# Jaureguy760/HaploHyped-VarAwareML

Measured on AMD Instinct MI355X. Metric: variants/sec encode+compress, 3M-variant x 2.5k-sample VCF, higher is better.
Workload: dtype u8

## Files before the change

### haplohyped_varawareml_amd/csrc/lz4bits.hip

```cpp
#include "common.h"

#define BP_N 4096
#ifndef BP_MAXONES
#define BP_MAXONES 636
#endif
#ifndef BP_STAGE
#define BP_STAGE 576
#endif
#ifndef BP_WAVES
#define BP_WAVES 7
#endif
#define BP_QCAP 100
#ifndef BP_MAXONES_EXC
#define BP_MAXONES_EXC 540
#endif
#ifndef BP_STAGE_EXC
#define BP_STAGE_EXC 448
#endif
template <bool EXC> struct BpCfg {
    static constexpr uint32_t MAXONES = EXC ? BP_MAXONES_EXC : BP_MAXONES;
    static constexpr uint32_t STAGE = EXC ? BP_STAGE_EXC : BP_STAGE;
    static constexpr uint32_t PTRASH = MAXONES + 7;
};
#define BP_HLOG 6
#define BP_GAPCLIP 40
#define BP_MINM 6
#define BP_TMIN 4
#define BP_BACK 64
#define BP_STEPS 16
#define BP_PICK 3
#define BP_LAZY_MIN 3
#ifdef BP_MARKS
#define BP_MARK(name) asm volatile("; ==MARK " name)
#else
#define BP_MARK(name)
#endif
#ifndef BP_SKIP
#define BP_SKIP 0
#endif
#define BP_MFLIMIT (BP_N - 12)
#define BP_MATCHLIMIT (BP_N - 5)

template <bool CHAIN, bool EXC> struct BpLds {
    uint32_t bm[132];
    uint32_t xm[EXC ? 132 : 1];
    uint32_t cls[EXC ? 24 : 1];
    uint32_t tab[1 << BP_HLOG];
    uint8_t flag[72];
    uint16_t wpre[64];
    uint16_t P[BpCfg<EXC>::MAXONES + 8];
    uint16_t chain[CHAIN ? BpCfg<EXC>::MAXONES + 8 : 4];
    uint32_t gbw[(BpCfg<EXC>::MAXONES + 16) / 4];
    uint2 queue[BP_QCAP + 1];
    uint8_t stage[BpCfg<EXC>::STAGE + 8];
};

__device__ __forceinline__ uint2 bp_entry(uint32_t E, uint32_t msr, bool onM, bool onT, uint32_t rs, uint32_t re, uint32_t off)
{
    return make_uint2(E | ((msr & 0x1FFFu) << 13) | (onM ? 1u << 26 : 0u) | (onT ? 1u << 27 : 0u) | ((rs - E) << 28), re | (off << 13));
}

__device__ __forceinline__ uint32_t bp_bits(const uint32_t *bm, uint32_t q)
{
    const uint32_t i = q >> 5;
    const uint32_t lo = bm[i], hi = bm[i + 1];
    return __builtin_amdgcn_alignbit(hi, lo, q & 31u);
}

__device__ __forceinline__ uint32_t bp_gap4(const uint32_t *gbw, uint32_t i)
{
    const uint32_t w = i >> 2;
    return __builtin_amdgcn_alignbit(gbw[w + 1u], gbw[w], (i & 3u) << 3);
}

__device__ __forceinline__ uint32_t bp_len_ext(uint32_t x) { return __umul24(x + 240u, 32897u) >> 23; }

template <bool EXC> __device__ __forceinline__ uint32_t bp_lit(uint32_t b, uint32_t x, uint32_t k)
{
    const uint32_t v = (b >> k) & 1u;
    return EXC ? (((x >> k) & 1u) ? 0xF7u : v) : v;
}

#define BP_FENCE() asm volatile("" ::: "memory")
#define BP_FORGET(x) asm volatile("" : "+v"(x))
#ifndef BP_EMITSKIP
#define BP_EMITSKIP 0
#endif
template <bool EXC, bool TR, typename OUT>
__device__ __forceinline__ void bp_put_entry(const uint32_t *bm, const uint32_t *xm, OUT out, uint32_t tr, uint32_t at, uint32_t pe, bool on1, uint32_t ll1,
                                             uint32_t ml1, uint32_t off1, bool on2, bool lit2, uint32_t ml2, uint32_t lane)
{
    if (BP_EMITSKIP == 3) return;
    const uint32_t llx1 = bp_len_ext(ll1), mlx1 = on1 ? bp_len_ext(ml1) : 0u, mlx2 = on2 ? bp_len_ext(ml2) : 0u, ll2 = lit2 ? 1u : 0u;
    auto put = [&](bool p, uint32_t a, uint32_t v) {
        if (TR) out[p ? a : tr] = (uint8_t)v;
        else if (p) out[a] = (uint8_t)v;
    };
    const uint32_t lit = at + 1u + llx1, o1 = lit + ll1;
    const uint32_t at2 = o1 + 2u + mlx1, o2 = at2 + 1u + ll2;
    if (__builtin_expect(__builtin_amdgcn_ballot_w64((llx1 > 1u) | (mlx1 > 1u) | (mlx2 > 1u)) != 0ull, 0)) {
        auto more = [&](uint32_t a, uint32_t v, uint32_t nx) {
            uint32_t r = v - 15u - 255u;
#pragma clang loop unroll(disable) vectorize(disable) interleave(disable)
            for (uint32_t k = 1; k < nx; ++k) {
                out[a + k] = (uint8_t)(k + 1u == nx ? r : 255u);
                r -= 255u;
            }
        };
        more(at + 1u, ll1, llx1);
        more(o1 + 2u, ml1, mlx1);
        more(o2 + 2u, ml2, mlx2);
    }
    put(on2, at2, (ll2 << 4) | (ml2 < 15u ? ml2 : 15u));
    put(lit2, at2 + 1u, 0u);
    put(on2, o2, 1u);
    put(on2, o2 + 1u, 0u);
    put(mlx2 != 0u, o2 + 2u, mlx2 == 1u ? ml2 - 15u : 255u);
    put(on1, at, ((ll1 < 15u ? ll1 : 15u) << 4) | (ml1 < 15u ? ml1 : 15u));
    put(llx1 != 0u, at + 1u, llx1 == 1u ? ll1 - 15u : 255u);
    put(on1, o1, off1 & 0xFFu);
    put(on1, o1 + 1u, off1 >> 8);
    put(mlx1 != 0u, o1 + 2u, mlx1 == 1u ? ml1 - 15u : 255u);
    if (BP_EMITSKIP != 1) {
        const uint32_t b = bp_bits(bm, pe), x = EXC ? bp_bits(xm, pe) : 0u;
        const uint32_t nsm = ll1 <= 6u ? ll1 : 0u;
#pragma unroll
        for (uint32_t k = 0; k < 6u; ++k) put(k < nsm, lit + k, bp_lit<EXC>(b, x, k));
        unsigned long long big = BP_EMITSKIP == 2 ? 0ull : __builtin_amdgcn_ballot_w64(ll1 > 6u);
        while (big != 0ull) {
            const int l = __builtin_ctzll(big);
            big &= big - 1ull;
            const uint32_t n = (uint32_t)__builtin_amdgcn_readlane((int)ll1, l);
            const uint32_t src = (uint32_t)__builtin_amdgcn_readlane((int)pe, l);
            const uint32_t dst = (uint32_t)__builtin_amdgcn_readlane((int)lit, l);
            for (uint32_t k = lane; k < n; k += 64u) out[dst + k] = (uint8_t)bp_lit<EXC>(bp_bits(bm, src + k), EXC ? bp_bits(xm, src + k) : 0u, 0u);
        }
    }
}

__device__ __forceinline__ void bp_flush(const uint8_t *stage, uint8_t *__restrict__ dst, uint32_t n, uint32_t lane)
{
    struct __attribute__((packed)) PU32 {
        uint32_t v;
    };
    const uint32_t nd = n >> 2;
    for (uint32_t i = lane; i < nd; i += 64u) reinterpret_cast<PU32 *>(dst + 4u * i)->v = reinterpret_cast<const uint32_t *>(stage)[i];
    const uint32_t t = (nd << 2) + lane;
    if (t < n) dst[t] = stage[t];
}

struct BpOut {
    uint32_t prev_end, gop, sop;
};

template <bool EXC, typename LDS>
__device__ __forceinline__ BpOut bp_emit_batch(LDS &S, const uint32_t *bm, uint8_t *__restrict__ out, uint32_t n, uint32_t qn, BpOut st, uint32_t lane)
{
    const uint32_t *xm = S.xm;
    uint32_t prev_end = st.prev_end, gop = st.gop, sop = st.sop;
    const bool have = lane < n;
    uint2 en = S.queue[lane];
    en.x = have ? en.x : 0u;
    en.y = have ? en.y : 0u;
    const uint32_t E = en.x & 0x1FFFu, msr = (en.x >> 13) & 0x1FFFu, rs = E + (en.x >> 28), re = en.y & 0x1FFFu, off = en.y >> 13;
    const bool onM = (en.x >> 26) & 1u;
    bool onT = (en.x >> 27) & 1u;
    {
        uint32_t nx = S.queue[lane + 1u].x;
        nx = lane + 1u < qn ? nx : 0u;
        const uint32_t nmsr = (nx >> 13) & 0x1FFFu;
        const bool nM = (nx >> 26) & 1u;
        uint32_t nbk = nM && nmsr <= re ? re - nmsr : 0u;
        const uint32_t zt = re - rs;
        nbk = nbk < zt ? nbk : zt;
        onT = onT && zt - nbk >= BP_TMIN;
    }
    const uint32_t F0 = onT ? re : E;
    uint32_t Fp = (uint32_t)__builtin_amdgcn_update_dpp(0, (int)F0, 0x138 , 0xf, 0xf, false);
    Fp = lane ? Fp : prev_end;
    const uint32_t F = (onM || onT) ? F0 : Fp;
    uint32_t pe = (uint32_t)__builtin_amdgcn_update_dpp(0, (int)F, 0x138 , 0xf, 0xf, false);
    pe = lane ? pe : prev_end;
    prev_end = (uint32_t)__builtin_amdgcn_readlane((int)F, (int)(n - 1u));
    const uint32_t ms = msr > pe ? msr : pe;
    const bool on1 = onM | onT, on2 = onM & onT;
    const uint32_t s1 = onM ? ms : rs, e1 = onM ? E : re;
    uint32_t ll1 = on1 ? s1 - pe : 0u, ml1 = e1 - s1 - 4u;
    const uint32_t off1 = onM ? off : 1u;
    const bool lit2 = on2 & (rs != E);
    uint32_t ml2 = re - rs - 4u;
    const uint32_t sz = (on1 ? 3u + bp_len_ext(ll1) + ll1 + bp_len_ext(ml1) : 0u) + (on2 ? 3u + (lit2 ? 1u : 0u) + bp_len_ext(ml2) : 0u);
    const uint32_t sincl = wave_scan_sum_dpp(sz, lane);
    const uint32_t total = (uint32_t)__builtin_amdgcn_readlane((int)sincl, 63);
    BP_MARK("sizes_done");
    if (__builtin_expect(sop + total > BpCfg<EXC>::STAGE, 0)) {
        bp_flush(S.stage, out + gop, sop, lane);
        gop += sop;
        sop = 0;
    }
    const uint32_t at = sincl - sz;
    BP_FORGET(ll1);
    BP_FORGET(ml1);
    BP_FORGET(ml2);
    if (__builtin_expect(total > BpCfg<EXC>::STAGE, 0)) {
        bp_put_entry<EXC, false>(bm, xm, out + gop, 0u, at, pe, on1, ll1, ml1, off1, on2, lit2, ml2, lane);
        gop += total;
    } else {
        bp_put_entry<EXC, true>(bm, xm, S.stage + sop, BpCfg<EXC>::STAGE - sop, at, pe, on1, ll1, ml1, off1, on2, lit2, ml2, lane);
        sop += total;
    }
    return BpOut{prev_end, gop, sop};
}


__device__ __forceinline__ void bp_probe_salu()
{
#ifdef BP_PROBE_SALU
#pragma unroll
    for (int pr = 0; pr < BP_PROBE_SALU; ++pr) asm volatile("s_mov_b32 s90, 0" ::: "s90");
#endif
}

__device__ __forceinline__ void bp_probe_valu()
{
#ifdef BP_PROBE_VALU
    uint32_t pv;
#pragma unroll
    for (int pr = 0; pr < BP_PROBE_VALU; ++pr) asm volatile("v_mov_b32 %0, 0" : "=v"(pv));
#endif
}

__device__ __forceinline__ uint32_t bp_probe_handoff(uint8_t *__restrict__ scratch, uint64_t sidx, uint64_t slot_bytes, uint32_t op, uint32_t lane)
{
#ifdef BP_PROBE_HANDOFF
    asm volatile("s_waitcnt vmcnt(0)" ::: "memory");
    uint32_t old = 0;
    if (lane == 0) old = atomicAdd(reinterpret_cast<uint32_t *>(scratch + (sidx & ~255ull) * slot_bytes + slot_bytes - 8u), 1u);
    old = (uint32_t)__builtin_amdgcn_readfirstlane((int)old);
    op += old == 0xFFFFFFF0u ? 1u : 0u;
#endif
    return op;
}

template <bool EXC, typename LDS>
__device__ __forceinline__ uint32_t bp_list_half(LDS &S, uint16_t *P, uint32_t w, uint32_t x, uint32_t at, uint32_t base)
{
    while (__builtin_amdgcn_ballot_w64(w != 0u) != 0ull) {
        const bool on = w != 0u;
        const uint32_t bpos = (uint32_t)__builtin_ctz(w | 0x80000000u);
        if (EXC && on && ((x >> bpos) & 1u)) atomicOr(&S.cls[at >> 5], 1u << (at & 31u));
        P[on ? at : BpCfg<EXC>::PTRASH] = (uint16_t)(base + bpos);
        at += on ? 1u : 0u;
        w &= w - 1u;
    }
    return at;
}

template <bool EXC, typename LDS>
__device__ __forceinline__ void bp_list_ones(LDS &S, uint16_t *P, uint16_t *wpre, uint32_t wlo, uint32_t whi, uint32_t xlo, uint32_t xhi, uint32_t incl,
                                             uint32_t cnt, uint32_t m, uint32_t lane)
{
    wpre[lane] = (uint16_t)(incl - cnt);
    BP_FENCE();
    P[lane == 0u ? 0u : BpCfg<EXC>::PTRASH] = 0;
    const uint32_t base = 64u * lane + 1u;
    const uint32_t at = bp_list_half<EXC>(S, P, wlo, xlo, incl - cnt + 1u, base);
    bp_list_half<EXC>(S, P, whi, xhi, at, base + 32u);
    P[lane < 4u ? m + 1u + lane : BpCfg<EXC>::PTRASH] = (uint16_t)(BP_N + 1);
    BP_FENCE();
}

template <bool EXC, typename LDS>
__device__ __forceinline__ void bp_gap_bytes(LDS &S, const uint16_t *P, uint32_t m, uint32_t lane)
{
    uint8_t *gb = reinterpret_cast<uint8_t *>(S.gbw);
    for (uint32_t i = lane; i < m + 8u; i += 64u) {
        const uint32_t i1 = i + 1u < BpCfg<EXC>::PTRASH ? i + 1u : BpCfg<EXC>::PTRASH;
        uint32_t g = (uint32_t)P[i1] - (uint32_t)P[i1 - 1u] - 1u;
        g = g < 255u ? g : 255u;
        gb[i] = (uint8_t)(i < m ? g : 255u);
    }
    BP_FENCE();
}

template <typename LDS>
__device__ __forceinline__ void bp_clear_table(LDS &S, uint32_t lane)
{
#pragma unroll
    for (int k = 0; k < (1 << BP_HLOG) / 64; ++k) S.tab[64 * k + lane] = 0u;
}

struct BpOne {
    int j, q;
    uint32_t jj, q1, qn1, qp1;
    uint32_t c5a;
    bool valid, can;
};

template <int DEPTH, bool EXC, typename LDS>
__device__ __forceinline__ BpOne bp_lane_one(LDS &S, const uint16_t *P, int jw, uint32_t m, uint32_t lane)
{
    BpOne o;
    o.j = jw + (int)lane;
    o.valid = o.j < (int)m;
    o.jj = o.valid ? (uint32_t)(o.j + 1) : 0u;
    o.q1 = P[o.jj], o.qn1 = P[o.jj + 1u];
    o.qp1 = o.jj ? P[o.jj - 1u] : 0u;
    o.q = (int)o.q1 - 1;
    o.can = DEPTH > 0 && o.valid && o.j >= 0 && o.q + 12 <= BP_N;
    o.c5a = EXC ? (bp_bits(S.cls, o.jj) & 31u) : 0u;
    return o;
}

template <bool CHAIN, bool EXC, typename LDS>
__device__ __forceinline__ uint32_t bp_table_insert(LDS &S, BpOne o)
{
    uint32_t jc1 = 0;
    if (o.can) {
        const uint32_t g1 = o.qn1 - o.q1;
        const uint32_t idx = (g1 < BP_GAPCLIP ? g1 : BP_GAPCLIP) ^ ((EXC && (o.c5a & 1u)) ? 63u : 0u);
        jc1 = atomicExch(&S.tab[idx], (uint32_t)(o.j + 1));
        if (CHAIN) S.chain[o.jj] = (uint16_t)jc1;
    }
    BP_FENCE();
    return jc1;
}

struct BpPick {
    int best;
    uint32_t bjq, bk;
    uint32_t a4;
};

template <int DEPTH, bool EXC, typename LDS>
__device__ __forceinline__ BpPick bp_pick(LDS &S, bool can, uint32_t jj, uint32_t c5a, uint32_t jc1)
{
    constexpr bool CHAIN = DEPTH > 1;
    const uint32_t a4 = bp_gap4(S.gbw, jj);
    const uint8_t *gbb = reinterpret_cast<const uint8_t *>(S.gbw);
    const uint32_t fa = jj ? (uint32_t)gbb[jj - 1u] : 0u;
    const uint32_t na4 = ~a4;
    const uint32_t stop4 = ((na4 - 0x01010101u) & ~na4 & 0x80808080u) | 0xFF000000u;
    int best = -1;
    uint32_t bjq = 0, bk = 0;
#pragma unroll 1
    for (int left = DEPTH; left > 0; --left) {
        const bool have = can && jc1 != 0u;
        if (__builtin_amdgcn_ballot_w64(have) == 0ull) break;
        const uint32_t jq = have ? jc1 : 1u;
        const uint32_t b4 = bp_gap4(S.gbw, jq);
        const uint32_t fb = (uint32_t)gbb[jq - 1u];
        uint32_t nextc = 0;
        if (CHAIN) nextc = S.chain[jq];
        const uint32_t x = (a4 ^ b4) | stop4;
        uint32_t k = (uint32_t)__builtin_ctz(x) >> 3;
        bool same = true;
        if (EXC) {
            const uint32_t xc = c5a ^ (bp_bits(S.cls, jq) & 31u);
            same = (xc & 1u) == 0u;
            const uint32_t tv = (uint32_t)__builtin_ctz((xc >> 1) | 8u);
            k = k < tv ? k : tv;
        }
        const uint32_t below = (1u << (8u * k)) - 1u;
        const uint32_t sumg = __builtin_amdgcn_sad_u8(a4 & below, 0u, k + 1u);
        const uint32_t za = (a4 >> (8u * k)) & 0xFFu, zb = (b4 >> (8u * k)) & 0xFFu;
        uint32_t fz = fa < fb ? fa : fb;
        fz = fz < BP_BACK ? fz : BP_BACK;
        const int score = (int)(sumg + (za < zb ? za : zb) + fz);
        const bool up = have & same & (score > best);
        best = up ? score : best;
        bjq = up ? jq : bjq;
        bk = up ? k : bk;
        if (!CHAIN) break;
        jc1 = have ? nextc : 0u;
    }
    return BpPick{best, bjq, bk, a4};
}

struct BpMatch {
    bool hv;
    uint32_t len, nb;
    uint32_t c1;
    uint32_t a_last;
    uint32_t z_last;
    bool clamped;
};

template <bool EXC, typename LDS>
__device__ __forceinline__ BpMatch bp_extend_and_price(LDS &S, const uint16_t *P, bool got, uint32_t bjq, uint32_t bk, uint32_t a4, uint32_t jj, int q,
                                                       uint32_t q1, uint32_t qp1, uint32_t m)
{
    uint32_t len = 0, nb = 0, c1 = 0, a_last = jj, z_last = 0;
    bool hv = false, clamped = false;
    if (__builtin_amdgcn_ballot_w64(got) != 0ull) {
        const uint32_t jq = got ? bjq : 1u;
        const uint32_t cc1 = P[jq], cp1 = P[jq - 1u];
        uint32_t a = jj + bk, b = jq + bk;
        uint32_t pa = P[a], pb = P[b];
        uint32_t clen = pa - q1, costR = 0, tailz = 0, zl = 0;
#pragma unroll
        for (uint32_t s = 0; s < BP_PICK; ++s) {
            const uint32_t g = (a4 >> (8u * s)) & 0xFFu;
            costR += s < bk ? 1u + (g >= BP_TMIN + 1u ? 4u : g) : 0u;
        }
        bool act = got;
        for (uint32_t s = bk;; ++s) {
            if (__builtin_amdgcn_ballot_w64(act) == 0ull) break;
            const uint32_t na = P[a + 1u], nbn = P[b + 1u];
            const uint32_t ga = na - pa - 1u, gb = nbn - pb - 1u;
            const bool cdiff = EXC && (((bp_bits(S.cls, a + 1u) ^ bp_bits(S.cls, b + 1u)) & 1u) != 0u);
            const bool stop = (s < BP_PICK) | (ga != gb) | (ga >= 255u) | (a >= m) | (s >= BP_STEPS) | cdiff;
            const uint32_t z = ga < gb ? ga : gb;
            costR += act ? 1u + (ga >= BP_TMIN + 1u ? 4u : ga) : 0u;
            clen += act ? 1u + (stop ? z : ga) : 0u;
            tailz = (act & stop) ? ga - z : tailz;
            zl = (act & stop) ? z : zl;
            act = act & !stop;
            a += act ? 1u : 0u;
            b += act ? 1u : 0u;
            pa = act ? na : pa;
            pb = act ? nbn : pb;
        }
        const uint32_t gq = q1 - qp1 - 1u, gc = cc1 - cp1 - 1u;
        uint32_t cnb = gq < gc ? gq : gc;
        cnb = cnb < BP_BACK ? cnb : BP_BACK;
        const uint32_t costH = 3u + (clen + cnb >= 19u ? 1u : 0u) - cnb + (tailz >= BP_TMIN ? 3u : tailz);
        uint32_t end = (uint32_t)q + clen;
        const bool cut = end > BP_MATCHLIMIT;
        end = end < BP_MATCHLIMIT ? end : BP_MATCHLIMIT;
        const int gain = (int)costR - (int)costH;
        hv = got & (gain > 0) & ((int)end - q >= 4) & ((int)end - (q - (int)cnb) >= BP_MINM) & (q <= BP_MFLIMIT);
        len = hv ? end - (uint32_t)q : 0u;
        nb = hv ? cnb : 0u;
        c1 = hv ? cc1 : 0u;
        a_last = a;
        z_last = zl;
        clamped = cut & hv;
    }
    return BpMatch{hv, len, nb, c1, a_last, z_last, clamped};
}

__device__ __forceinline__ BpMatch bp_lazy_rule(bool hv, uint32_t len, uint32_t nb, uint32_t c1, uint32_t a_last, uint32_t z_last, bool clamped, int j, int q,
                                             uint32_t jj, uint32_t q1, uint32_t qn1, uint32_t m, uint32_t lane)
{
    const uint32_t E0 = hv ? (uint32_t)q + len : (uint32_t)(q + 1);
    const uint32_t hvN = (uint32_t)__builtin_amdgcn_update_dpp(0, (int)(hv ? 1u : 0u), 0x130 , 0xf, 0xf, false);
    const uint32_t EN = (uint32_t)__builtin_amdgcn_update_dpp(0, (int)E0, 0x130, 0xf, 0xf, false);
    const uint32_t nbN = (uint32_t)__builtin_amdgcn_update_dpp(0, (int)nb, 0x130, 0xf, 0xf, false);
    const int msN = (int)qn1 - 1 - (int)nbN;
    const int between = msN - (int)q1 > 0 ? msN - (int)q1 : 0;
    const bool Ln = hv & (hvN != 0u) & (lane < 63u) & (j + 1 < (int)m) & (qn1 <= E0) &
                    ((int)EN - (int)E0 >= (int)(BP_LAZY_MIN + nb) + between);
    const unsigned long long lm = __builtin_amdgcn_ballot_w64(Ln);
    const unsigned long long rest = ~(lm >> lane);
    const uint32_t tlo = (uint32_t)__builtin_ctz((uint32_t)rest | 0x80000000u), thi = (uint32_t)__builtin_ctz((uint32_t)(rest >> 32) | 0x80000000u);
    const uint32_t t = (uint32_t)rest != 0u ? tlo : 32u + thi;
    const bool give = Ln && (t & 1u);
    return BpMatch{hv && !give, give ? 0u : len, give ? 0u : nb, give ? 0u : c1, give ? jj : a_last, give ? 0u : z_last, clamped && !give};
}

struct BpNext {
    uint32_t E;
    uint32_t nxt;
};

__device__ __forceinline__ BpNext bp_next_one(const uint32_t *bm, const uint16_t *wpre, bool hv, uint32_t len, uint32_t a_last, bool clamped, int q, uint32_t jj,
                                           uint32_t m)
{
    const uint32_t E = hv ? (uint32_t)q + len : (uint32_t)(q + 1);
    uint32_t nxt = hv ? a_last : jj;
    if (__builtin_amdgcn_ballot_w64(clamped) != 0ull) {
        const uint32_t w = E >> 6, bb = E & 63u, wc = w < 63u ? w : 63u;
        const uint32_t lo = bm[2u * wc], hi = bm[2u * wc + 1u];
        const uint32_t mlo = bb >= 32u ? 0xFFFFFFFFu : ((1u << bb) - 1u);
        const uint32_t mhi = bb > 32u ? ((1u << (bb - 32u)) - 1u) : 0u;
        const uint32_t in_map = (uint32_t)wpre[wc] + (uint32_t)__popc(lo & mlo) + (uint32_t)__popc(hi & mhi);
        nxt = clamped ? (w >= 64u ? m : in_map) : nxt;
    }
    return BpNext{E, nxt};
}

struct BpSel {
    bool sel;
    int cur;
};

__device__ __forceinline__ BpSel bp_select_coded(uint8_t *flag, bool valid, uint32_t nxt, int jw, int cur, uint32_t lane)
{
    bool sel = false;
    if (cur < jw + 64) {
        const uint32_t e0 = (uint32_t)(cur - jw);
        uint32_t jump = valid ? (nxt - (uint32_t)jw < 64u ? nxt - (uint32_t)jw : 64u) : 64u;
        const uint32_t p0 = jump;
        flag[lane] = lane == e0 ? 1u : 0u;
        flag[lane == 0u ? 64u : 69u] = 0u;
        BP_FENCE();
        bool reach = lane == e0;
#pragma unroll
        for (int r = 0; r < 6; ++r) {
            flag[reach ? jump : 68u] = 1u;
            BP_FENCE();
            reach = flag[lane] != 0u;
            const uint32_t j2 = (uint32_t)__builtin_amdgcn_ds_bpermute((int)((jump & 63u) << 2), (int)jump);
            jump = jump < 64u ? j2 : 64u;
        }
        sel = reach && valid;
        const unsigned long long ex = __builtin_amdgcn_ballot_w64(sel && p0 == 64u);
        if (ex != 0ull) cur = (int)__builtin_amdgcn_readlane((int)nxt, (int)(__ffsll((long long)ex) - 1));
    }
    return BpSel{sel, cur};
}

struct BpQueued {
    BpOut out;
    uint32_t qn;
};

template <bool EXC, typename LDS>
__device__ __forceinline__ BpQueued bp_queue_and_drain(LDS &S, const uint32_t *bm, const uint16_t *P, uint8_t *out, int q, uint32_t q1, bool hv, uint32_t nb,
                                                       uint32_t c1, uint32_t z_last, bool clamped, uint32_t E, uint32_t nxt, bool sel, int jw, uint32_t m,
                                                       uint32_t prev_end, uint32_t gop, uint32_t sop, uint32_t qn, uint32_t lane)
{
    const bool onM = sel && hv;
    uint32_t rs = E + ((!hv || z_last == 0u) ? 1u : 0u);
    if (__builtin_amdgcn_ballot_w64(clamped) != 0ull)
        rs = clamped ? E + ((bp_bits(bm, E - 1u) & 1u) ? 1u : 0u) : rs;
    uint32_t re = (uint32_t)P[(nxt < m ? nxt : m) + 1u] - 1u;
    re = re < BP_MATCHLIMIT ? re : BP_MATCHLIMIT;
    const bool onT = sel && (int)re - (int)rs >= BP_TMIN && rs <= BP_MFLIMIT;
    const bool want = onM || onT;
    const unsigned long long wm = __builtin_amdgcn_ballot_w64(want);
    const uint32_t nw = (uint32_t)__builtin_popcountll(wm);
    const bool last = jw + 64 >= (int)m;
    const uint2 ent = bp_entry(E, (uint32_t)(q - (int)nb), onM, onT, rs, re, q1 - c1);
    for (int phase = 0; phase < 2; ++phase) {
        if (phase == 1) {
            const uint32_t slot = qn + __builtin_amdgcn_mbcnt_hi((uint32_t)(wm >> 32), __builtin_amdgcn_mbcnt_lo((uint32_t)wm, 0u));
            S.queue[want ? slot : (uint32_t)BP_QCAP] = ent;
            qn += nw;
            BP_MARK("queued");
        }
        while (phase == 0 ? qn + nw > BP_QCAP : (qn >= 65u || (last && qn != 0u))) {
            const uint32_t keep = phase == 1 && last ? 0u : 1u;
            const uint32_t nb_ = qn - keep < 64u ? qn - keep : 64u;
            BP_FENCE();
            const BpOut r = bp_emit_batch<EXC>(S, bm, out, nb_, qn, BpOut{prev_end, gop, sop}, lane);
            prev_end = r.prev_end, gop = r.gop, sop = r.sop;
            BP_FENCE();
            const bool mvp = lane + nb_ < qn;
            const uint2 mv = S.queue[mvp ? nb_ + lane : (uint32_t)BP_QCAP];
            BP_FENCE();
            S.queue[mvp ? lane : (uint32_t)BP_QCAP] = mv;
            qn -= nb_;
        }
    }
    return BpQueued{BpOut{prev_end, gop, sop}, qn};
}

template <bool EXC, typename LDS>
__device__ __forceinline__ BpOut bp_last_literals(LDS &S, const uint32_t *bm, uint8_t *out, uint32_t prev_end, uint32_t gop, uint32_t sop, uint32_t lane)
{
    const uint32_t ll = BP_N - prev_end, llx = bp_len_ext(ll);
    BP_FENCE();
    if (sop + 1u + llx + ll > BpCfg<EXC>::STAGE) {
        bp_flush(S.stage, out + gop, sop, lane);
        gop += sop;
        sop = 0;
    }
    const bool direct = 1u + llx + ll > BpCfg<EXC>::STAGE;
    auto tail = [&](auto dstp) {
        if (lane == 0) {
            dstp[0] = (uint8_t)((ll < 15u ? ll : 15u) << 4);
            uint32_t r = ll - 15u;
            for (uint32_t k = 0; k < llx; ++k) {
                dstp[1u + k] = (uint8_t)(k + 1u == llx ? r : 255u);
                r -= 255u;
            }
        }
        for (uint32_t k = lane; k < ll; k += 64u)
            dstp[1u + llx + k] = (uint8_t)bp_lit<EXC>(bp_bits(bm, prev_end + k), EXC ? bp_bits(S.xm, prev_end + k) : 0u, 0u);
    };
    if (direct) {
        tail(out + gop);
        gop += 1u + llx + ll;
    } else {
        tail(S.stage + sop);
        sop += 1u + llx + ll;
    }
    return BpOut{prev_end, gop, sop};
}

template <bool EXC, typename LDS>
__device__ __forceinline__ uint32_t bp_finish_stream(LDS &S, const uint32_t *bm, uint8_t *out, BpOut st, uint32_t lane)
{
    uint32_t op = st.gop + st.sop;
    if (op >= BP_N) {
        for (uint32_t k = lane; k < BP_N; k += 64u) out[k] = (uint8_t)bp_lit<EXC>(bp_bits(bm, k), EXC ? bp_bits(S.xm, k) : 0u, 0u);
        op = BP_N;
    } else {
        BP_FENCE();
        bp_flush(S.stage, out + st.gop, st.sop, lane);
    }
    return op;
}

template <int DEPTH, bool EXC, bool LAZY, typename LDS>
__device__ __forceinline__ void bp_code_plane(LDS &S, uint32_t wlo, uint32_t whi, uint32_t xlo, uint32_t xhi, bool nonbinary, uint32_t bid,
                                              uint32_t wave, uint32_t lane, uint8_t *__restrict__ scratch, uint64_t slot_bytes,
                                              uint32_t *__restrict__ csize, uint32_t *__restrict__ flags, uint32_t tag)
{
    uint32_t sink = 0;
    uint32_t *bm = S.bm;
    uint16_t *P = S.P;
    uint16_t *wpre = S.wpre;
    uint8_t *flag = S.flag;
    const uint64_t sidx = (uint64_t)bid * 2u + wave;
    uint8_t *out = scratch + sidx * slot_bytes;

    const uint32_t cnt = (uint32_t)__popc(wlo) + (uint32_t)__popc(whi);
    uint32_t m;
    const uint32_t incl = wave_scan_sum_dpp(cnt, lane, &m);
    if (nonbinary || m > BpCfg<EXC>::MAXONES) {
        if (lane == 0 && flags && flags[0] != tag) flags[0] = tag;
        if (lane == 0) csize[sidx] = 0xFFFFFFFFu;
        return;
    }
    BP_MARK("scan_done");
    bp_list_ones<EXC>(S, P, wpre, wlo, whi, xlo, xhi, incl, cnt, m, lane);
    if (DEPTH > 0) bp_gap_bytes<EXC>(S, P, m, lane);
    bp_clear_table(S, lane);
    BP_MARK("plist_done");
    if (BP_SKIP >= 4) {
        if (lane == 0) csize[sidx] = P[m] & 1u;
        return;
    }
    BpQueued st{BpOut{0u, 0u, 0u}, 0u};
    int cur = -1;
    for (int jw = -1; jw < (int)m; jw += 64) {
        BP_MARK("win_begin");
        bp_probe_salu();
        bp_probe_valu();
        const BpOne o = bp_lane_one<DEPTH, EXC>(S, P, jw, m, lane);
        const uint32_t jc1 = bp_table_insert<(DEPTH > 1), EXC>(S, o);
        BP_MARK("hash_done");
        BpMatch mt{false, 0u, 0u, 0u, o.jj, 0u, false};
        if (DEPTH > 0) {
            const BpPick pk = bp_pick<DEPTH, EXC>(S, o.can, o.jj, o.c5a, jc1);
            mt = bp_extend_and_price<EXC>(S, P, pk.best >= 0, pk.bjq, pk.bk, pk.a4, o.jj, o.q, o.q1, o.qp1, m);
        }
        BP_MARK("cand_done");
        if (LAZY) mt = bp_lazy_rule(mt.hv, mt.len, mt.nb, mt.c1, mt.a_last, mt.z_last, mt.clamped, o.j, o.q, o.jj, o.q1, o.qn1, m, lane);
        const BpNext nx = bp_next_one(bm, wpre, mt.hv, mt.len, mt.a_last, mt.clamped, o.q, o.jj, m);
        BP_MARK("nxt_done");
        if (BP_SKIP >= 3) {
            sink += nx.nxt + nx.E;
            continue;
        }
        const BpSel sl = bp_select_coded(flag, o.valid, nx.nxt, jw, cur, lane);
        cur = sl.cur;
        BP_MARK("sel_done");
        if (BP_SKIP >= 2) {
            sink += sl.sel ? nx.nxt : 0u;
            continue;
        }
        st = bp_queue_and_drain<EXC>(S, bm, P, out, o.q, o.q1, mt.hv, mt.nb, mt.c1, mt.z_last, mt.clamped, nx.E, nx.nxt, sl.sel, jw, m, st.out.prev_end,
                                     st.out.gop, st.out.sop, st.qn, lane);
        BP_MARK("emit_done");
    }
    BP_MARK("loop_done");
    if (BP_SKIP >= 1) {
        if (lane == 0) csize[sidx] = (st.out.prev_end + sink) & 0xFFFu;
        return;
    }
    uint32_t op = bp_finish_stream<EXC>(S, bm, out, bp_last_literals<EXC>(S, bm, out, st.out.prev_end, st.out.gop, st.out.sop, lane), lane);
    if (BP_SKIP) op = (op & 0xFFFu) + (sink & 1u);
    op = bp_probe_handoff(scratch, sidx, slot_bytes, op, lane);
    if (lane == 0) csize[sidx] = op;
}

template <int DEPTH, bool LAZY = false>
__global__ __launch_bounds__(128, BP_WAVES) void k_lz4_bitplanes(const uint8_t *__restrict__ src, PlanesGeom pg, uint32_t n_blocks,
                                                                  uint8_t *__restrict__ scratch, uint64_t slot_bytes, uint32_t *__restrict__ csize,
                                                                  uint32_t *__restrict__ flags, uint32_t tag)
{
    constexpr bool CHAIN = DEPTH > 1;
    __shared__ BpLds<CHAIN, false> lds[2];
    __shared__ uint32_t nonbin[2][2];
    const uint32_t wave = (uint32_t)__builtin_amdgcn_readfirstlane((int)(threadIdx.x >> 6)), lane = threadIdx.x & 63u;
    const uint32_t bid = blockIdx.x;
    for (int once = 0; once < 1; ++once) {
    const uint8_t *blk = src + (uint64_t)bid * 8192u;

    {
        typedef uint32_t u32x4 __attribute__((ext_vector_type(4)));
        const u32x4 *p = reinterpret_cast<const u32x4 *>(blk + 4096u * wave + 16u * lane);
        u32x4 v[4];
#pragma unroll
        for (int k = 0; k < 4; ++k) v[k] = __builtin_nontemporal_load(p + 64 * k);
        uint32_t orall = 0;
        uint8_t *bm0 = reinterpret_cast<uint8_t *>(lds[0].bm) + 256u * wave + lane;
        uint8_t *bm1 = reinterpret_cast<uint8_t *>(lds[1].bm) + 256u * wave + lane;
#pragma unroll
        for (int k = 0; k < 4; ++k) {
            const uint32_t d[4] = {v[k].x, v[k].y, v[k].z, v[k].w};
            uint32_t acc0 = 0, acc1 = 0;
#pragma unroll
            for (int i = 0; i < 4; ++i) {
                const uint32_t x = d[i];
                orall |= x;
                const uint32_t xm = x & 0x01010101u;
                const uint32_t y = xm | (xm >> 15);
                acc0 |= (y & 3u) << (2 * i);
                acc1 |= ((y >> 8) & 3u) << (2 * i);
            }
            bm0[64 * k] = (uint8_t)acc0;
            bm1[64 * k] = (uint8_t)acc1;
        }
        const uint32_t nb0 = orall & 0x00FE00FEu, nb1 = orall & 0xFE00FE00u;
        const unsigned long long b0 = __builtin_amdgcn_ballot_w64(nb0 != 0u), b1 = __builtin_amdgcn_ballot_w64(nb1 != 0u);
        if (lane == 0) {
            nonbin[wave][0] = b0 != 0ull;
            nonbin[wave][1] = b1 != 0ull;
        }
        if (lane < 4u) lds[wave].bm[128u + lane] = 0u;
    }
    __syncthreads();
    const uint32_t wlo = lds[wave].bm[2u * lane], whi = lds[wave].bm[2u * lane + 1u];
    const bool nonbinary = (nonbin[0][wave] | nonbin[1][wave]) != 0u;
    BP_MARK("A_done");
    if (BP_SKIP >= 5) {
        if (lane == 0) csize[(uint64_t)bid * 2u + wave] = lds[wave].bm[5] & 1u;
        return;
    }

    bp_code_plane<DEPTH, false, LAZY>(lds[wave], wlo, whi, 0u, 0u, nonbinary, bid, wave, lane, scratch, slot_bytes, csize, flags, tag);
    }
}

template <int DEPTH, bool LAZY>
__global__ __launch_bounds__(128, BP_WAVES) void k_lz4_bitplanes_uni(const uint8_t *__restrict__ src, PlanesGeom pg, uint32_t n_blocks,
                                                                      uint8_t *__restrict__ scratch, uint64_t slot_bytes,
                                                                      uint32_t *__restrict__ csize, uint32_t *__restrict__ flags, uint32_t tag)
{
    constexpr bool CHAIN = DEPTH > 1;
    union BpBoth {
        BpLds<CHAIN, false> p;
        BpLds<CHAIN, true> x;
    };
    __shared__ BpBoth lds[2];
    const uint32_t wave = (uint32_t)__builtin_amdgcn_readfirstlane((int)(threadIdx.x >> 6)), lane = threadIdx.x & 63u;
    const uint32_t bid = (blockIdx.x & ~63u) | ((blockIdx.x & 7u) << 3) | ((blockIdx.x >> 3) & 7u);
    if (bid >= n_blocks) return;
    typedef uint32_t u32x2 __attribute__((ext_vector_type(2)));
    uint64_t col;
    uint32_t row, bi;
    planes_block(pg, bid, &col, &row, &bi);
    const u32x2 *pl = reinterpret_cast<const u32x2 *>(src + planes_piece(pg, col, bi * 16u + (lane >> 2), wave, row)) + (lane & 3u);
    const u32x2 one = *pl, exc = *(pl + (uint64_t)pg.S_pad * 8ull);
    if (__builtin_amdgcn_ballot_w64((exc.x | exc.y) != 0u) == 0ull) {
        BpLds<CHAIN, false> &S = lds[wave].p;
        S.bm[2u * lane] = one.x;
        S.bm[2u * lane + 1u] = one.y;
        if (lane < 4u) S.bm[128u + lane] = 0u;
        bp_code_plane<DEPTH, false, LAZY>(S, one.x, one.y, 0u, 0u, false, bid, wave, lane, scratch, slot_bytes, csize, flags, tag);
    } else {
        BpLds<CHAIN, true> &S = lds[wave].x;
        const bool nonbinary = __builtin_amdgcn_ballot_w64(((exc.x & ~one.x) | (exc.y & ~one.y)) != 0u) != 0ull;
        S.bm[2u * lane] = one.x;
        S.bm[2u * lane + 1u] = one.y;
        if (lane < 4u) S.bm[128u + lane] = 0u;
        S.xm[2u * lane] = exc.x;
        S.xm[2u * lane + 1u] = exc.y;
        if (lane < 4u) S.xm[128u + lane] = 0u;
        if (lane < 24u) S.cls[lane] = 0u;
        bp_code_plane<DEPTH, true, LAZY>(S, one.x, one.y, exc.x, exc.y, nonbinary, bid, wave, lane, scratch, slot_bytes, csize, flags, tag);
    }
}

template <int D, bool LZ>
static void bp_launch(bool planes, const uint8_t *d_src, PlanesGeom pg, uint32_t n_blocks, uint8_t *d_scratch, uint64_t slot_bytes, uint32_t *d_csize,
                      uint32_t *d_flags, uint32_t tag, hipStream_t st)
{
    if (planes)
        hipLaunchKernelGGL((k_lz4_bitplanes_uni<D, LZ>), dim3((n_blocks + 63u) / 64u * 64u), dim3(128), 0, st, d_src, pg, n_blocks, d_scratch, slot_bytes,
                           d_csize, d_flags, tag);
    else
        hipLaunchKernelGGL((k_lz4_bitplanes<D, LZ>), dim3(n_blocks), dim3(128), 0, st, d_src, pg, n_blocks, d_scratch, slot_bytes, d_csize, d_flags, tag);
}

int launch_lz4_bitplanes(const uint8_t *d_src, bool planes, PlanesGeom pg, uint64_t n_blocks, uint8_t *d_scratch, size_t slot_bytes, uint32_t *d_csize,
                         int depth, uint32_t *d_flags, uint32_t tag, hipStream_t st)
{
    const bool lazy = (depth & 0x100) != 0;
    depth &= 0xFF;
    if (n_blocks == 0) return HHGT_OK;
    if (n_blocks > 0x7fffffffull) {
        hhgt_set_error("lz4: too many blocks");
        return HHGT_ERR_ARG;
    }
    const auto launch = lazy ? (depth == 2 ? bp_launch<2, true> : bp_launch<12, true>)
                        : depth <= 0 ? bp_launch<0, false>
                        : depth == 1 ? bp_launch<1, false>
                        : depth == 2 ? bp_launch<2, false>
                        : depth <= 4 ? bp_launch<4, false>
                        : depth <= 8 ? bp_launch<8, false>
                        : depth <= 12 ? bp_launch<12, false>
                                      : bp_launch<16, false>;
    launch(planes, d_src, pg, (uint32_t)n_blocks, d_scratch, (uint64_t)slot_bytes, d_csize, d_flags, tag, st);
    HIP_TRY(hipGetLastError());
    return HHGT_OK;
}
```

Before: 160.0 million.

## Split bitplane LZ4 kernel into one-wave workgroups and shrink LDS staging

Result: faster. 169.7 million (median of 6 runs) (+6.1%).

```diff
diff --git a/haplohyped_varawareml_amd/csrc/lz4bits.hip b/haplohyped_varawareml_amd/csrc/lz4bits.hip
--- a/haplohyped_varawareml_amd/csrc/lz4bits.hip
+++ b/haplohyped_varawareml_amd/csrc/lz4bits.hip
@@ -4,24 +4,32 @@
 #ifndef BP_MAXONES
 #define BP_MAXONES 636
 #endif
+#ifndef BP_QCAP
+#define BP_QCAP 80
+#endif
 #ifndef BP_STAGE
-#define BP_STAGE 576
+#define BP_STAGE 240
 #endif
 #ifndef BP_WAVES
 #define BP_WAVES 7
 #endif
-#define BP_QCAP 100
 #ifndef BP_MAXONES_EXC
 #define BP_MAXONES_EXC 540
 #endif
+#ifndef BP_QCAP_EXC
+#define BP_QCAP_EXC 80
+#endif
 #ifndef BP_STAGE_EXC
-#define BP_STAGE_EXC 448
-#endif
+#define BP_STAGE_EXC 104
+#endif
+#define BP_PLANE_LDS 5120
 template <bool EXC> struct BpCfg {
     static constexpr uint32_t MAXONES = EXC ? BP_MAXONES_EXC : BP_MAXONES;
+    static constexpr uint32_t QCAP = EXC ? BP_QCAP_EXC : BP_QCAP;
     static constexpr uint32_t STAGE = EXC ? BP_STAGE_EXC : BP_STAGE;
     static constexpr uint32_t PTRASH = MAXONES + 7;
 };
+static_assert(BP_QCAP >= 65 && BP_QCAP_EXC >= 65, "a batch of 64 needs the entry behind it in the queue");
 #define BP_HLOG 6
 #define BP_GAPCLIP 40
 #define BP_MINM 6
@@ -51,7 +59,7 @@
     uint16_t P[BpCfg<EXC>::MAXONES + 8];
     uint16_t chain[CHAIN ? BpCfg<EXC>::MAXONES + 8 : 4];
     uint32_t gbw[(BpCfg<EXC>::MAXONES + 16) / 4];
-    uint2 queue[BP_QCAP + 1];
+    uint2 queue[BpCfg<EXC>::QCAP + 1];
     uint8_t stage[BpCfg<EXC>::STAGE + 8];
 };
 
@@ -536,11 +544,11 @@
     for (int phase = 0; phase < 2; ++phase) {
         if (phase == 1) {
             const uint32_t slot = qn + __builtin_amdgcn_mbcnt_hi((uint32_t)(wm >> 32), __builtin_amdgcn_mbcnt_lo((uint32_t)wm, 0u));
-            S.queue[want ? slot : (uint32_t)BP_QCAP] = ent;
+            S.queue[want ? slot : BpCfg<EXC>::QCAP] = ent;
             qn += nw;
             BP_MARK("queued");
         }
-        while (phase == 0 ? qn + nw > BP_QCAP : (qn >= 65u || (last && qn != 0u))) {
+        while (phase == 0 ? qn + nw > BpCfg<EXC>::QCAP : (qn >= 65u || (last && qn != 0u))) {
             const uint32_t keep = phase == 1 && last ? 0u : 1u;
             const uint32_t nb_ = qn - keep < 64u ? qn - keep : 64u;
             BP_FENCE();
@@ -548,9 +556,9 @@
             prev_end = r.prev_end, gop = r.gop, sop = r.sop;
             BP_FENCE();
             const bool mvp = lane + nb_ < qn;
-            const uint2 mv = S.queue[mvp ? nb_ + lane : (uint32_t)BP_QCAP];
+            const uint2 mv = S.queue[mvp ? nb_ + lane : BpCfg<EXC>::QCAP];
             BP_FENCE();
-            S.queue[mvp ? lane : (uint32_t)BP_QCAP] = mv;
+            S.queue[mvp ? lane : BpCfg<EXC>::QCAP] = mv;
             qn -= nb_;
         }
     }
@@ -738,18 +746,20 @@
 }
 
 template <int DEPTH, bool LAZY>
-__global__ __launch_bounds__(128, BP_WAVES) void k_lz4_bitplanes_uni(const uint8_t *__restrict__ src, PlanesGeom pg, uint32_t n_blocks,
-                                                                      uint8_t *__restrict__ scratch, uint64_t slot_bytes,
-                                                                      uint32_t *__restrict__ csize, uint32_t *__restrict__ flags, uint32_t tag)
+__global__ __launch_bounds__(64, BP_WAVES) void k_lz4_bitplanes_uni(const uint8_t *__restrict__ src, PlanesGeom pg, uint32_t n_blocks,
+                                                                     uint8_t *__restrict__ scratch, uint64_t slot_bytes,
+                                                                     uint32_t *__restrict__ csize, uint32_t *__restrict__ flags, uint32_t tag)
 {
     constexpr bool CHAIN = DEPTH > 1;
     union BpBoth {
         BpLds<CHAIN, false> p;
         BpLds<CHAIN, true> x;
     };
-    __shared__ BpBoth lds[2];
-    const uint32_t wave = (uint32_t)__builtin_amdgcn_readfirstlane((int)(threadIdx.x >> 6)), lane = threadIdx.x & 63u;
-    const uint32_t bid = (blockIdx.x & ~63u) | ((blockIdx.x & 7u) << 3) | ((blockIdx.x >> 3) & 7u);
+    static_assert(sizeof(BpBoth) <= BP_PLANE_LDS, "32 planes per CU");
+    __shared__ BpBoth lds;
+    const uint32_t lane = threadIdx.x;
+    const uint32_t r = blockIdx.x & 127u, k = r >> 3;
+    const uint32_t bid = (blockIdx.x >> 7) * 64u + (r & 7u) * 8u + (k >> 1), wave = k & 1u;
     if (bid >= n_blocks) return;
     typedef uint32_t u32x2 __attribute__((ext_vector_type(2)));
     uint64_t col;
@@ -758,13 +768,13 @@
     const u32x2 *pl = reinterpret_cast<const u32x2 *>(src + planes_piece(pg, col, bi * 16u + (lane >> 2), wave, row)) + (lane & 3u);
     const u32x2 one = *pl, exc = *(pl + (uint64_t)pg.S_pad * 8ull);
     if (__builtin_amdgcn_ballot_w64((exc.x | exc.y) != 0u) == 0ull) {
-        BpLds<CHAIN, false> &S = lds[wave].p;
+        BpLds<CHAIN, false> &S = lds.p;
         S.bm[2u * lane] = one.x;
         S.bm[2u * lane + 1u] = one.y;
         if (lane < 4u) S.bm[128u + lane] = 0u;
         bp_code_plane<DEPTH, false, LAZY>(S, one.x, one.y, 0u, 0u, false, bid, wave, lane, scratch, slot_bytes, csize, flags, tag);
     } else {
-        BpLds<CHAIN, true> &S = lds[wave].x;
+        BpLds<CHAIN, true> &S = lds.x;
         const bool nonbinary = __builtin_amdgcn_ballot_w64(((exc.x & ~one.x) | (exc.y & ~one.y)) != 0u) != 0ull;
         S.bm[2u * lane] = one.x;
         S.bm[2u * lane + 1u] = one.y;
@@ -782,7 +792,7 @@
                       uint32_t *d_flags, uint32_t tag, hipStream_t st)
 {
     if (planes)
-        hipLaunchKernelGGL((k_lz4_bitplanes_uni<D, LZ>), dim3((n_blocks + 63u) / 64u * 64u), dim3(128), 0, st, d_src, pg, n_blocks, d_scratch, slot_bytes,
+        hipLaunchKernelGGL((k_lz4_bitplanes_uni<D, LZ>), dim3((n_blocks + 63u) / 64u * 128u), dim3(64), 0, st, d_src, pg, n_blocks, d_scratch, slot_bytes,
                            d_csize, d_flags, tag);
     else
         hipLaunchKernelGGL((k_lz4_bitplanes<D, LZ>), dim3(n_blocks), dim3(128), 0, st, d_src, pg, n_blocks, d_scratch, slot_bytes, d_csize, d_flags, tag);
@@ -794,7 +804,7 @@
     const bool lazy = (depth & 0x100) != 0;
     depth &= 0xFF;
     if (n_blocks == 0) return HHGT_OK;
-    if (n_blocks > 0x7fffffffull) {
+    if (2u * n_blocks > 0x7fffff80ull) {
         hhgt_set_error("lz4: too many blocks");
         return HHGT_ERR_ARG;
     }
```
